# indrajeetadityaroy9/vit-inductive-bias-distillation

Hardware: AMD Instinct MI355X
Metric: distillation images/sec (BASD loss fwd+bwd+grad all-reduce), DeiT-S<-ResNet-50 @ bs256/GPU (higher is better)
Workload: dtype f32; 1 GPU; cfg2 DeiT-S<-ResNet-50 224x224; per_gpu_batch=256, global_batch=256, input_dtype=float32, layout=strided (CLS-sliced / channel-major views), backward=True, grad_allreduce_bytes=88202672, grad_allreduce=none at world size 1 (bucket packed, nothing to exchange), rank_readback=auto, readback_deferred_steps=1756, selector=basd_selector_chain mode 0, parallelism=dp1

## Files before the change

include/basd_hip.h:

```cpp
#ifndef BASD_HIP_H
#define BASD_HIP_H

#include <stdint.h>

#ifdef __cplusplus
extern "C" {
#endif

#ifndef __HIP_PLATFORM_AMD__
typedef struct ihipStream_t* hipStream_t;
#endif

#define BASD_OK 0
#define BASD_EINVAL (-1)
#define BASD_EUNSUPPORTED (-2)
#define BASD_DTYPE_F32 0
#define BASD_DTYPE_BF16 1
#define BASD_DTYPE_U8 2


int basd_gemm_nt(const void* a, int a_dtype, long a_sb, long a_sn, long a_sd, int a_rows_per_batch,
                 long a_batch_stride, const float* b, long ldb, long b_batch_stride, int M, int N, int K, int batch,
                 float* c, long ldc, long c_batch_stride, float scale, const float* bias, float beta,
                 float* colsum_part, float* col_mean, hipStream_t stream);
// ... 196 lines not shown
    const void* const* attn_ptrs;
    long a_dtype, a_sb, a_sh, a_sq, a_sk;
    const float* mix;
    long E, L, G, B, n_s, n_t, d_s, d_t, H, A, has_cls, n_a, n, max_sweeps;
    const int* atap0; const int* atap1; const float* alam;
    const int* tap0; const int* tap1; const float* lam; const int* range0; const int* range1;
    const int* g0; const int* g1; const float* glam;
    float* omega; float* omega_t; float* raw; float* mu_t; float* tc; float* mu_s; float* tr_part; float* tr_s;
    float* a_prime;
    double* g_all; double* l_all;
    float* W; float* sigma; int* jflags; int* sweeps;
    float* tr_t; float* nuc; float* loss_b; float* k_prime;
    float* h; float* dx; const float* grad_layers;
    double* g_slabs; long g_splits;
    const float* uw_ce; float* uw_out;
    void* jac_ws;
    float* w_stack; float* sigma_u;
} BasdProcrustesArgs;
int basd_procrustes_forward_fused(const BasdProcrustesArgs* args, hipStream_t stream);
int basd_procrustes_tuning(int transposed_cores);

int basd_stack_product_t(const double* la, const double* lb, long l_batch_stride, int n, int batch, int lb_period,
                         float* w, long w_batch_stride, hipStream_t stream);
int basd_kprime_from_transposed(const float* w, long w_batch_stride, const float* sigma, int n, int batch,
                                const double* lb, long l_batch_stride, int lb_period, float* z, long z_batch_stride,
                                float* k_prime, hipStream_t stream);
int basd_procrustes_finish_transposed(const float* w, long w_batch_stride, const float* sigma, int n, int n_s,
                                      int batch, int t_period ,
                                      const double* gb, long g_batch_stride, const float* omega, const int* tap0,
                                      const int* tap1, const float* lam, const float* tr_s_part, int tr_slabs,
                                      float* tr_s, float* tr_t, float* nuc, float* loss, const double* lb,
                                      long l_batch_stride, int lb_period, float* k_prime, hipStream_t stream);
int basd_procrustes_finish_tuning(int fused);
int basd_ustack_stash(const float* wc, long wc_batch_stride, int n, int batch, float* w_stack, long w_stack_stride,
                      hipStream_t stream);
int basd_ustack_from_transposed(const float* x, long x_batch_stride, const float* sigma, int n, int batch,
                                float* w_stack, long w_stack_stride, float* scratch, long scratch_batch_stride,
                                float* sigma_u, int max_sweeps, int* jflags, hipStream_t stream);

int basd_scale_unless_one(float* x, long count, const float* num, const float* den, hipStream_t stream);

int basd_cross_entropy(const void* logits, int dtype, long ld, int B, int C, const long* labels, const float* probs,
                       long pld, float label_smoothing, long ignore_index, float* row_loss, float* dlogits,
                       hipStream_t stream);


int basd_event_create(void** out);
int basd_event_destroy(void* event);
int basd_stream_wait_event(hipStream_t stream, void* event);
int basd_event_record(void* event, hipStream_t stream);
int basd_event_synchronize(void* event);
int basd_stream_create_priority(void** out, int level);
int basd_event_create_timed(void** out);
int basd_event_elapsed_ms(void* from, void* to, float* ms_out);


int basd_teacher_factor(const float* w, long w_batch_stride, const float* sigma, int n, int n_s, int batch,
                        const double* la, const double* gb, long g_batch_stride, const float* omega,
                        const int* tap0, const int* tap1, const float* lam, const int* range0, const int* range1,
                        float* kt, float* tnorm2, hipStream_t stream);
int basd_teacher_factor_tiled(const float* w, long w_batch_stride, const float* sigma, int n, int n_s, int batch,
                              const double* la, const double* gb, long g_batch_stride, const float* omega,
                              const int* tap0, const int* tap1, const float* lam, const int* range0, const int* range1,
                              float* kt, float* tnorm2, float* z_scratch, hipStream_t stream);

int basd_mix_grad_tokens(const float* r, const void* const* tok_ptrs, int dtype, int L, long sb, long sn, long sd,
// ... 89 lines not shown
```

vit-inductive-bias-distillation_amd/basd_amd/_lib.py:

```python
from __future__ import annotations

import ctypes as C
import os
import threading

_HERE = os.path.dirname(os.path.abspath(__file__))
LIB_PATH = os.path.join(_HERE, "libbasd_hip.so")

vp, i32, i64, f32, f64 = C.c_void_p, C.c_int, C.c_long, C.c_float, C.c_double

SIGNATURES = {
    "basd_gemm_nt": [vp, i32, i64, i64, i64, i32, i64, vp, i64, i64, i32, i32, i32, i32, vp, i64, i64, f32, vp, f32,
                     vp, vp, vp],
    "basd_gemm_tn_splits": [i32],
    "basd_gemm_tn": [vp, vp, i32, i64, i64, i64, i64, i64, i64, i64, i64, i32, i32, i32, i32, i32, vp, vp, i32, vp,
                     vp, i64, i64, f32, vp],
    "basd_colmean_parts": [i32],
    "basd_colmean": [vp, i32, i64, i64, i64, i32, i64, i32, i32, i32, i32, vp, vp, vp],
    "basd_colmean_multi": [vp, i32, i64, i64, i64, i32, i32, i32, i32, i32, vp, vp, i32, vp],
    "basd_syrk_splits": [i32, i32, i32],
    "basd_syrk_multi": [vp, i32, i64, i64, i64, i32, i32, i32, i32, vp, vp, i32, vp, vp, i64, i32, vp, i32, i32, vp],
    "basd_jacobi_workspace_ints": [i32, i32],
    "basd_jacobi_twopass_workspace_bytes": [i32, i32, i32],
    "basd_jacobi_stacked_twopass": [vp, i64, i32, i32, vp, i32, i32, f32, vp, vp, vp],
# ... 23 lines not shown
    "basd_grassmann_distance": [vp, i32, vp, vp, i32, vp, i32, vp, vp, vp],
    "basd_grassmann_distance_padded": [vp, i32, i32, vp, vp, i32, vp, i32, vp, vp],
    "basd_selector_tail": [vp] * 10 + [i32, i32, i32, i32] + [vp] * 14 + [vp],
    "basd_sqrt_clamp": [vp, vp, i64, vp],
    "basd_gram_finish": [vp, vp, i32, i32, i64, vp, vp, vp],
    "basd_cross_entropy": [vp, i32, i64, i32, i32, vp, vp, i64, f32, i64, vp, vp, vp],
    "basd_token_weights": [vp, i32, vp, i32, i64, i64, i64, i64, i32, i32, i32, i32, i32, i32, i32, vp, vp, vp, vp,
                           vp, vp, vp, vp, vp, vp],
    "basd_student_project": [vp, i32, i64, i64, i32, i32, i32, i32, vp, vp, vp, vp, vp, vp, vp, vp, vp, vp],
    "basd_teacher_center": [vp, i32, vp, i32, i64, i64, i64, i32, i32, i32, vp, vp, vp, vp, vp, vp, vp],
    "basd_teacher_center_multi": [vp, i32, vp, i32, i32, i64, i64, i64, i32, i32, i32, vp, vp, vp, vp, vp, vp, vp],
    "basd_teacher_center_stream_scratch_floats": [i32, i32, i32, i32],
    "basd_teacher_center_stream": [vp, i32, vp, i32, i32, i64, i64, i64, i32, i32, i32, vp, vp, vp, vp, vp, vp, vp, vp],
    "basd_gram_f64": [vp, i64, i32, i32, i32, vp, i64, vp],
    "basd_gram_f64_split": [vp, i64, i32, i32, i32, i32, vp, vp, vp],
    "basd_chol_f64": [vp, i64, i32, i32, vp, i64, vp],
    "basd_stack_product": [vp, vp, i64, i32, i32, i32, vp, i64, vp],
    "basd_procrustes_finalize": [vp, i64, vp, i32, i32, i32, i32, vp, i64, vp, vp, vp, vp, vp, i32, vp, vp, vp, vp,
                                 vp, vp],
    "basd_student_project_multi": [vp, i32, i64, i64, i32, i32, i32, i32, i32, i32, vp, i64, vp, vp, vp, vp, vp, vp,
                                   vp, vp, vp],
    "basd_student_grad_multi": [vp, i32, i64, i64, i32, i32, i32, i32, i32, vp, i64, vp, vp, vp, vp, vp, vp, f32, vp,
                                vp, vp, vp],
    "basd_student_grad_fused": [vp, i32, i64, i64, i32, i32, i32, i32, i32, i32, vp, i64, vp, vp, vp, vp, vp, vp, vp,
                                f32, vp, vp],
    "basd_procrustes_forward_fused": [vp, vp],
    "basd_procrustes_tuning": [i32],
    "basd_jacobi_plain4_fits": [i32],
    "basd_stack_product_t": [vp, vp, i64, i32, i32, i32, vp, i64, vp],
    "basd_kprime_from_transposed": [vp, i64, vp, i32, i32, vp, i64, i32, vp, i64, vp, vp],
    "basd_procrustes_finish_transposed": [vp, i64, vp, i32, i32, i32, i32, vp, i64, vp, vp, vp, vp, vp, i32, vp, vp, vp,
                                          vp, vp, i64, i32, vp, vp],
    "basd_procrustes_finish_tuning": [i32],
    "basd_ustack_stash": [vp, i64, i32, i32, vp, i64, vp],
    "basd_ustack_from_transposed": [vp, i64, vp, i32, i32, vp, i64, vp, i64, vp, i32, vp, vp],
    "basd_resample_tokens": [vp, i32, i64, i64, i64, i32, i32, i32, i32, vp, vp, vp, vp, vp],
    "basd_resample_tokens_adjoint": [vp, i32, i32, i32, i32, vp, vp, vp, vp, vp, vp, vp],
    "basd_teacher_factor": [vp, i64, vp, i32, i32, i32, vp, vp, i64, vp, vp, vp, vp, vp, vp, vp, vp, vp],
    "basd_teacher_factor_tiled": [vp, i64, vp, i32, i32, i32, vp, vp, i64, vp, vp, vp, vp, vp, vp, vp, vp, vp, vp],
    "basd_mix_grad_tokens": [vp, vp, i32, i32, i64, i64, i64, i32, i32, i32, i32, vp, vp, vp, vp, vp],
    "basd_mix_grad_tokens_scratch_floats": [i32, i32, i32, i32],
    "basd_mix_grad_tokens_onepass": [vp, vp, i32, i32, i64, i64, i64, i32, i32, i32, i32, vp, vp, vp, vp, vp, vp],
    "basd_token_weight_bwd": [vp, vp, i32, i32, i32, i32, vp, vp, vp, vp, vp, vp, i32, i32, i64, i64, i64, i64, i32,
                              i32, i32, vp, vp, vp],
    "basd_build_angle_stack": [vp, i32, vp, i32, vp, vp],
    "basd_grassmann_distance_bwd": [vp, vp, i32, vp, vp, i32, vp, vp, i32, vp, vp],
    "basd_eigvec_k2": [vp, vp, i32, i32, i32, vp, vp],
    "basd_selector_chain": [vp],
    "basd_rank_certificate": [vp, vp, i32, i32, f64, vp, vp, vp],
    "basd_rank_certificate_scratch_bytes": [i32],
    "basd_debug_fill_lds": [C.c_uint, vp],
    "basd_selector_chain_tail": [vp, i32, i32],
    "basd_jacobi_lds_square_fits": [i32],
    "basd_event_record": [vp, vp],
    "basd_event_synchronize": [vp],
    "basd_stream_create_priority": [vp, i32],
    "basd_event_create_timed": [vp],
    "basd_event_elapsed_ms": [vp, vp, vp],
    "basd_sfadamw_chunk": [],
    "basd_sfadamw_step": [vp, vp, i32, vp, i32, f32, i32, vp],
    "basd_sfadamw_swap": [vp, vp, i32, vp, i32, vp],
    "basd_sfadamw_launches": [],
    "basd_eval_batch": [vp, i32, i64, i32, i32, vp, i32, vp, f32, i32, vp, vp],
    "basd_mix_batch": [vp, i32, vp, i32, i32, i32, i32, i32, i32, f64, i32, i32, i32, i32, vp, vp, vp, i32, f64, vp,
                       vp],
    "basd_attn_importance": [vp, i32, i64, i64, i32, i32, i32, i32, i32, f32, vp, vp],
# ... 94 lines not shown
```

vit-inductive-bias-distillation_amd/csrc/fused.hip:

```cpp
#include "basd_common.h"
#include "../../include/basd_hip.h"

namespace basd {

__global__ void __launch_bounds__(256) uwso_combine_kernel(const float* __restrict__ ce, const float* __restrict__ loss_b,
                                                           int E, int B, float* __restrict__ out) {
    constexpr int CH = 32;
    __shared__ double red[CH][4];
    const int tid = threadIdx.x;
    double geo_sum = 0.;
    for (int e0 = 0; e0 < E; e0 += CH) {
        const int ne = E - e0 < CH ? E - e0 : CH;
        for (int e = 0; e < ne; ++e) {
            double acc = 0.;
            for (int b = tid; b < B; b += 256) acc += (double)loss_b[(long)(e0 + e) * B + b];
            for (int m = 32; m > 0; m >>= 1) acc += __shfl_xor(acc, m, 64);
            if ((tid & 63) == 0) red[e][tid >> 6] = acc;
        }
        __syncthreads();
        if (tid == 0)
            for (int e = 0; e < ne; ++e) {
                const float layer = (float)(((red[e][0] + red[e][1]) + (red[e][2] + red[e][3])) / (double)B);
                out[4 + E + e0 + e] = layer;
                geo_sum += (double)layer;
            }
        __syncthreads();
    }
    if (tid == 0) {
        const float c = ce[0], geo = (float)(geo_sum / (double)E);
        const float eps = 1.1920929e-7f;
        const float i0 = 1.f / fmaxf(c, eps), i1 = 1.f / fmaxf(geo, eps);
        const float w0 = i0 / (i0 + i1), w1 = i1 / (i0 + i1);
        out[0] = w0;
        out[1] = w1;
        out[2] = w0 * c + w1 * geo;
        out[3] = geo;
        for (int e = 0; e < E; ++e) out[4 + e] = w1 / (float)E;
    }
}

__global__ void __launch_bounds__(256) scale_unless_one_kernel(float* __restrict__ x, long count4, long count,
                                                               const float* __restrict__ num,
                                                               const float* __restrict__ den) {
    const float f = den ? num[0] / den[0] : num[0];
    if (f == 1.f) return;
    const long i = (long)blockIdx.x * 256 + threadIdx.x;
    if (i < count4) {
        float4 v = ((float4*)x)[i];
        v.x *= f; v.y *= f; v.z *= f; v.w *= f;
        ((float4*)x)[i] = v;
    }
    if (blockIdx.x == 0 && threadIdx.x < (int)(count - 4 * count4)) x[4 * count4 + threadIdx.x] *= f;
}

}

extern "C" {

int basd_scale_unless_one(float* x, long count, const float* num, const float* den, hipStream_t stream) {
    BASD_CHECK_ARG(x && num && count > 0 && ((uintptr_t)x & 15) == 0);
    const long count4 = count / 4;
    basd::scale_unless_one_kernel<<<(unsigned)((count4 + 255) / 256 + (count4 == 0)), 256, 0, stream>>>(x, count4, count, num, den);
    BASD_RETURN_LAST();
}

static int procrustes_tail(const BasdProcrustesArgs* a, const float* grad_layers, int E, int B, int n_s, int n, int d_s,
                           int EB, long nn, long om_stride, hipStream_t st) {
    int rc;
#define BASD_TRY(call)            \
    do {                          \
        rc = (call);              \
        if (rc != BASD_OK) return rc; \
    } while (0)
    if (a->uw_ce) {
        BASD_CHECK_ARG(a->uw_out != nullptr);
        basd::uwso_combine_kernel<<<1, 256, 0, st>>>(a->uw_ce, a->loss_b, E, B, a->uw_out);
        grad_layers = a->uw_out + 4;
    }
    if (a->dx) {
        BASD_CHECK_ARG(a->k_prime && a->h && grad_layers);
        rc = basd_student_grad_fused(a->student_ptrs, (int)a->s_dtype, a->s_sb, a->s_sn, E, B, n_s, n, d_s,
                                     (int)a->s_aligned, a->omega, om_stride, a->mu_s, a->k_prime, a->a_prime, a->tap0,
                                     a->tap1, a->lam, grad_layers, 2.0f / (float)B, a->dx, st);
        if (rc != BASD_EUNSUPPORTED) return rc;
        BASD_TRY(basd_gemm_tn(a->k_prime, a->a_prime, BASD_DTYPE_F32, 0, n, 1, nn, 0, d_s, 1, (long)n * d_s, 1 << 30, n,
                              n, d_s, EB, nullptr, nullptr, 1, nullptr, a->h, d_s, (long)n * d_s, 1.f, st));
        BASD_TRY(basd_student_grad_multi(a->student_ptrs, (int)a->s_dtype, a->s_sb, a->s_sn, E, B, n_s, n, d_s, a->omega,
                                         om_stride, a->mu_s, a->h, a->tap0, a->tap1, a->lam, grad_layers,
                                         2.0f / (float)B, a->dx, nullptr, nullptr, st));
    }
#undef BASD_TRY
    return BASD_OK;
}

static int g_transposed_cores = 1;
// ... 132 lines not shown
```

vit-inductive-bias-distillation_amd/csrc/procrustes.hip:

```cpp
#include "basd_common.h"
#include "../../include/basd_hip.h"

namespace basd {

typedef double f64x4 __attribute__((ext_vector_type(4)));

template <typename T>
__global__ void __launch_bounds__(256) token_weights_kernel(const void* const* __restrict__ attn_ptrs,
                                                            const float* __restrict__ mix, int L, long sb, long sh,
                                                            long sq, long sk, int H, int A, int has_cls, int n_a,
                                                            int n_t, int n_s, const int* __restrict__ atap0,
                                                            const int* __restrict__ atap1,
                                                            const float* __restrict__ alam,
                                                            const int* __restrict__ tap0,
                                                            const int* __restrict__ tap1,
                                                            const float* __restrict__ lam, float* __restrict__ omega,
                                                            float* __restrict__ omega_t, float* __restrict__ raw_out) {
    extern __shared__ float sm[];
    float* raw = sm;
    float* w = sm + n_a;
    __shared__ float red[32];
    const int b = blockIdx.x, tid = threadIdx.x;
    for (int j = tid; j < n_a; j += blockDim.x) {
        float acc = 0.f;
        if (has_cls) {
            for (int h = 0; h < H; ++h) {
                float m = 0.f;
                for (int l = 0; l < L; ++l)
                    m += mix[l] * ldg_f32((const BASD_GLOBAL_AS T*)attn_ptrs[l] + (b * sb + h * sh + (long)(1 + j) * sk));
                acc += m;
            }
            acc /= (float)H;
// ... 7 lines not shown
                }
            acc /= (float)(H * A);
        }
        raw[j] = acc;
        if (raw_out) raw_out[(long)b * n_a + j] = acc;
    }
    __syncthreads();
    float part = 0.f;
    for (int n = tid; n < n_s; n += blockDim.x) {
        float v;
        if (atap0) {
            const float l1 = alam[n];
            v = (1.f - l1) * raw[atap0[n]] + l1 * raw[atap1[n]];
        } else {
            v = raw[n];
        }
        w[n] = v;
        part += v;
    }
    const float total = block_sum(part, red);
    for (int n = tid; n < n_s; n += blockDim.x) {
        const float v = w[n] / total;
        w[n] = v;
        omega[(long)b * n_s + n] = v;
    }
    __syncthreads();
    for (int j = tid; j < n_t; j += blockDim.x) {
        float acc = 0.f;
        if (tap0) {
            for (int n = 0; n < n_s; ++n) {
                const float l1 = lam[n];
                if (tap0[n] == j) acc += (1.f - l1) * w[n];
                if (tap1[n] == j) acc += l1 * w[n];
            }
        } else {
            acc = w[j];
        }
        omega_t[(long)b * n_t + j] = acc;
    }
}

template <typename T>
__global__ void __launch_bounds__(256) student_project_kernel(const T* __restrict__ X, long sb, long sn, int n_s,
                                                              int n_t, int D, const float* __restrict__ omega,
                                                              const int* __restrict__ tap0,
                                                              const int* __restrict__ tap1,
                                                              const float* __restrict__ lam,
                                                              const int* __restrict__ range0,
                                                              const int* __restrict__ range1,
                                                              float* __restrict__ mu_out, float* __restrict__ tr_part,
                                                              float* __restrict__ Ap) {
    extern __shared__ float sm[];
    float* w = sm;
    __shared__ float red[4][64];
    __shared__ float mu[64];
    __shared__ float scratch[32];
    const int b = blockIdx.y, d0 = blockIdx.x * 64, tid = threadIdx.x;
    const int cl = tid & 63, rg = tid >> 6, d = d0 + cl;
    const bool live = d < D;
    const T* Xb = X + (long)b * sb + d;
    for (int n = tid; n < n_s; n += 256) w[n] = omega[(long)b * n_s + n];
    __syncthreads();
    float acc = 0.f;
    if (live)
        for (int n = rg; n < n_s; n += 4) acc = fmaf(w[n], to_f32(Xb[(long)n * sn]), acc);
    red[rg][cl] = acc;
// ... 165 lines not shown
    }
    *(float4*)(&red[rg][c4]) = acc;
    __syncthreads();
    if (tid < SP_W) {
        float m = 0.f;
#pragma unroll
        for (int q = 0; q < 32; ++q) m += red[q][tid];
        mu[tid] = m;
        if (d0 + tid < D) mu_out[((long)e * B + b) * D + d0 + tid] = m;
    }
    __syncthreads();
    const float4 m4 = *(const float4*)(mu + c4);
    float part = 0.f;
    if (live)
        for (int n = rg; n < n_s; n += 32) {
            const float4 v = *(const float4*)(xs + n * SP_W + c4);
            const float cx = v.x - m4.x, cy = v.y - m4.y, cz = v.z - m4.z, cw = v.w - m4.w;
            part = fmaf(w[n], fmaf(cx, cx, fmaf(cy, cy, fmaf(cz, cz, cw * cw))), part);
        }
    const float tr = block_sum(part, scratch);
    if (tid == 0) tr_part[((long)e * B + b) * gridDim.x + blockIdx.x] = tr;
    if (!live) return;
    float* Ab = Ap + ((long)e * B + b) * n_t * D + d0 + c4;
    for (int j = rg; j < n_t; j += 32) {
        const int n0 = range0 ? range0[j] : j, n1 = range1 ? range1[j] : j + 1;
        float4 a = make_float4(0.f, 0.f, 0.f, 0.f);
        for (int n = n0; n < n1; ++n) {
            const float cw = tap0 ? (t0[n] == j ? c0[n] : 0.f) + (t1[n] == j ? c1[n] : 0.f) : w[n];
            const float4 v = *(const float4*)(xs + n * SP_W + c4);
            a.x = fmaf(cw, v.x - m4.x, a.x); a.y = fmaf(cw, v.y - m4.y, a.y);
            a.z = fmaf(cw, v.z - m4.z, a.z); a.w = fmaf(cw, v.w - m4.w, a.w);
        }
        *(float4*)(Ab + (long)j * D) = a;
    }
}

template <typename T>
__global__ void __launch_bounds__(256) teacher_center_kernel(const void* const* __restrict__ tok_ptrs,
                                                             const float* __restrict__ mix, int L, long sb, long sn,
                                                             long sd, int n, int D, const int* __restrict__ g0,
                                                             const int* __restrict__ g1,
                                                             const float* __restrict__ glam,
                                                             const float* __restrict__ omega_t,
                                                             float* __restrict__ mu_out, float* __restrict__ Tc) {
    extern __shared__ float sm[];
    float* tile = sm;
    float* wt = sm + (size_t)n * 65;
    float* mu = wt + n;
    const int b = blockIdx.y, d0 = blockIdx.x * 64, tid = threadIdx.x;
    for (int j = tid; j < n; j += 256) wt[j] = omega_t[(long)b * n + j];
    const int total = n * 64;
    const bool feat_fast = sd == 1;
    for (int idx = tid; idx < total; idx += 256) {
        int j, dd;
        if (feat_fast) { j = idx >> 6; dd = idx & 63; }
        else { dd = idx / n; j = idx - dd * n; }
        const int d = d0 + dd;
        float v = 0.f;
        if (d < D) {
            const long off = b * sb + (long)d * sd;
            if (g0) {
                const long r0 = g0[j], r1 = g1[j];
                float a0 = 0.f, a1 = 0.f;
                for (int l = 0; l < L; ++l) {
                    const BASD_GLOBAL_AS T* p = (const BASD_GLOBAL_AS T*)tok_ptrs[l];
                    a0 = fmaf(mix[l], ldg_f32(p + (off + r0 * sn)), a0);
                    a1 = fmaf(mix[l], ldg_f32(p + (off + r1 * sn)), a1);
                }
                const float l1 = glam[j];
                v = (1.f - l1) * a0 + l1 * a1;
            } else {
                for (int l = 0; l < L; ++l)
                    v = fmaf(mix[l], ldg_f32((const BASD_GLOBAL_AS T*)tok_ptrs[l] + (off + (long)j * sn)), v);
            }
        }
        tile[j * 65 + dd] = v;
    }
    __syncthreads();
    if (tid < 64) {
        float acc = 0.f;
        for (int j = 0; j < n; ++j) acc = fmaf(wt[j], tile[j * 65 + tid], acc);
        mu[tid] = acc;
        if (d0 + tid < D) mu_out[(long)b * D + d0 + tid] = acc;
    }
    __syncthreads();
    float* out = Tc + (long)b * n * D;
    for (int idx = tid; idx < total; idx += 256) {
        const int j = idx >> 6, dd = idx & 63, d = d0 + dd;
        if (d < D) out[(long)j * D + d] = tile[j * 65 + dd] - mu[dd];
    }
}

constexpr int TCM_W = 16, TCM_G = 4;
template <typename T>
__global__ void __launch_bounds__(256) teacher_center_multi_kernel(
    const void* const* __restrict__ tok_ptrs, const float* __restrict__ mix, int L, int G, long sb, long sn, long sd,
    int n, int D, const int* __restrict__ g0, const int* __restrict__ g1, const float* __restrict__ glam,
    const float* __restrict__ omega_t, float* __restrict__ mu_out, float* __restrict__ Tc) {
    extern __shared__ float sm[];
    const int B = gridDim.y, b = blockIdx.y, d0 = blockIdx.x * TCM_W, tid = threadIdx.x;
    float* tile = sm;
    float* wt = sm + (size_t)G * n * (TCM_W + 1);
    float* mu = wt + (size_t)G * n;
    for (int idx = tid; idx < G * n; idx += 256) {
        const int g = idx / n, j = idx - g * n;
        wt[idx] = omega_t[((long)g * B + b) * n + j];
    }
    const int total = n * TCM_W;
    const bool feat_fast = sd == 1;
    for (int idx = tid; idx < total; idx += 256) {
        int j, dd;
        if (feat_fast) { j = idx / TCM_W; dd = idx - j * TCM_W; }
        else { dd = idx / n; j = idx - dd * n; }
        const int d = d0 + dd;
        float v[TCM_G] = {0.f, 0.f, 0.f, 0.f};
        if (d < D) {
            const long off = b * sb + (long)d * sd;
            if (g0) {
                const long r0 = g0[j], r1 = g1[j];
                const float l1 = glam[j], l0 = 1.f - l1;
                for (int l = 0; l < L; ++l) {
                    const BASD_GLOBAL_AS T* p = (const BASD_GLOBAL_AS T*)tok_ptrs[l];
                    const float x = l0 * ldg_f32(p + (off + r0 * sn)) + l1 * ldg_f32(p + (off + r1 * sn));
#pragma unroll
                    for (int g = 0; g < TCM_G; ++g)
// ... 922 lines not shown
    const T* x0 = X + (long)b * sb + (long)i0 * sn;
    const T* x1 = X + (long)b * sb + (long)i1 * sn;
    float* o = out + ((long)b * n_out + s) * D;
    for (int d = threadIdx.x; d < D; d += 128) o[d] = l0 * to_f32(x0[(long)d * sd]) + l1 * to_f32(x1[(long)d * sd]);
}

__global__ void __launch_bounds__(128) resample_tokens_adjoint_kernel(const float* __restrict__ dY, int n_in,
                                                                      int n_out, int D,
                                                                      const int* __restrict__ tap0,
                                                                      const int* __restrict__ tap1,
                                                                      const float* __restrict__ lam,
                                                                      const int* __restrict__ range0,
                                                                      const int* __restrict__ range1,
                                                                      float* __restrict__ dX) {
    const int j = blockIdx.x, b = blockIdx.y;
    const int s0 = range0[j], s1 = range1[j];
    for (int d = threadIdx.x; d < D; d += 128) {
        float acc = 0.f;
        for (int s = s0; s < s1; ++s) {
            const float l1 = lam[s];
            const float coef = (tap0[s] == j ? 1.f - l1 : 0.f) + (tap1[s] == j ? l1 : 0.f);
            acc = fmaf(coef, dY[((long)b * n_out + s) * D + d], acc);
        }
        dX[((long)b * n_in + j) * D + d] = acc;
    }
}

}

using namespace basd;

extern "C" {

int basd_token_weights(const void* const* attn_ptrs, int dtype, const float* mix, int L, long sb, long sh, long sq,
                       long sk, int B, int H, int A, int has_cls, int n_a, int n_t, int n_s, const int* atap0,
                       const int* atap1, const float* alam, const int* tap0, const int* tap1, const float* lam,
                       float* omega, float* omega_t, float* raw_out, hipStream_t stream) {
    BASD_CHECK_ARG(attn_ptrs && mix && omega && omega_t && L > 0 && B > 0 && H > 0 && n_a > 0 && n_t > 0 && n_s > 0);
    BASD_CHECK_ARG(A == n_a + (has_cls ? 1 : 0));
    BASD_CHECK_ARG((n_a == n_s) == (atap0 == nullptr));
    BASD_CHECK_ARG((n_t == n_s) == (tap0 == nullptr));
    const size_t lds = sizeof(float) * (size_t)(n_a + n_s);
    if (dtype == BASD_DTYPE_F32)
        token_weights_kernel<float><<<B, 256, lds, stream>>>(attn_ptrs, mix, L, sb, sh, sq, sk, H, A, has_cls, n_a, n_t, n_s, atap0, atap1, alam, tap0, tap1, lam, omega, omega_t, raw_out);
    else if (dtype == BASD_DTYPE_BF16)
        token_weights_kernel<__hip_bfloat16><<<B, 256, lds, stream>>>(attn_ptrs, mix, L, sb, sh, sq, sk, H, A, has_cls, n_a, n_t, n_s, atap0, atap1, alam, tap0, tap1, lam, omega, omega_t, raw_out);
    else
        return BASD_EINVAL;
    BASD_RETURN_LAST();
}

int basd_student_project(const void* x, int dtype, long sb, long sn, int B, int n_s, int n_t, int D,
                         const float* omega, const int* tap0, const int* tap1, const float* lam, const int* range0,
                         const int* range1, float* mu, float* tr_s, float* a_prime, hipStream_t stream) {
    BASD_CHECK_ARG(x && omega && mu && tr_s && a_prime && B > 0 && n_s > 0 && n_t > 0 && D > 0);
    BASD_CHECK_ARG((n_t == n_s) == (tap0 == nullptr));
    const size_t lds = sizeof(float) * (size_t)n_s;
    const dim3 grid((D + 63) / 64, B);
    const int esz = dtype == BASD_DTYPE_F32 ? 4 : 2;
    const size_t lds_slab = sizeof(float) * (size_t)n_s * 65;
    const bool staged = D % 4 == 0 && ((uintptr_t)x * 1) % 16 == 0 && (sb * esz) % 16 == 0 && (sn * esz) % 16 == 0 &&
                        (esz == 4 || D % 8 == 0) && lds_slab <= 64 * 1024;
    if (dtype == BASD_DTYPE_F32) {
        if (staged) {
            (void)hipFuncSetAttribute((const void*)student_project_lds_kernel<float>, hipFuncAttributeMaxDynamicSharedMemorySize, (int)lds_slab);
            student_project_lds_kernel<float><<<grid, 256, lds_slab, stream>>>((const float*)x, sb, sn, n_s, n_t, D, omega, tap0, tap1, lam, range0, range1, mu, tr_s, a_prime);
        } else {
            student_project_kernel<float><<<grid, 256, lds, stream>>>((const float*)x, sb, sn, n_s, n_t, D, omega, tap0, tap1, lam, range0, range1, mu, tr_s, a_prime);
        }
    } else if (dtype == BASD_DTYPE_BF16) {
        if (staged) {
            (void)hipFuncSetAttribute((const void*)student_project_lds_kernel<__hip_bfloat16>, hipFuncAttributeMaxDynamicSharedMemorySize, (int)lds_slab);
            student_project_lds_kernel<__hip_bfloat16><<<grid, 256, lds_slab, stream>>>((const __hip_bfloat16*)x, sb, sn, n_s, n_t, D, omega, tap0, tap1, lam, range0, range1, mu, tr_s, a_prime);
        } else {
            student_project_kernel<__hip_bfloat16><<<grid, 256, lds, stream>>>((const __hip_bfloat16*)x, sb, sn, n_s, n_t, D, omega, tap0, tap1, lam, range0, range1, mu, tr_s, a_prime);
        }
    } else {
        return BASD_EINVAL;
    }
    BASD_RETURN_LAST();
}

int basd_teacher_center(const void* const* tok_ptrs, int dtype, const float* mix, int L, long sb, long sn, long sd,
                        int B, int n, int D, const int* g0, const int* g1, const float* glam, const float* omega_t,
                        float* mu, float* tc, hipStream_t stream) {
    BASD_CHECK_ARG(tok_ptrs && mix && omega_t && mu && tc && L > 0 && B > 0 && n > 0 && D > 0);
    BASD_CHECK_ARG((g0 == nullptr) == (g1 == nullptr) && (g0 == nullptr) == (glam == nullptr));
    const size_t lds = sizeof(float) * ((size_t)n * 65 + n + 64);
    if (lds > 150 * 1024) return BASD_EUNSUPPORTED;
    const dim3 grid((D + 63) / 64, B);
    if (dtype == BASD_DTYPE_F32) {
        (void)hipFuncSetAttribute((const void*)teacher_center_kernel<float>, hipFuncAttributeMaxDynamicSharedMemorySize, 150 * 1024);
        teacher_center_kernel<float><<<grid, 256, lds, stream>>>(tok_ptrs, mix, L, sb, sn, sd, n, D, g0, g1, glam, omega_t, mu, tc);
    } else if (dtype == BASD_DTYPE_BF16) {
        (void)hipFuncSetAttribute((const void*)teacher_center_kernel<__hip_bfloat16>, hipFuncAttributeMaxDynamicSharedMemorySize, 150 * 1024);
        teacher_center_kernel<__hip_bfloat16><<<grid, 256, lds, stream>>>(tok_ptrs, mix, L, sb, sn, sd, n, D, g0, g1, glam, omega_t, mu, tc);
    } else {
        return BASD_EINVAL;
    }
    BASD_RETURN_LAST();
}

int basd_teacher_center_multi(const void* const* tok_ptrs, int dtype, const float* mix, int L, int G, long sb, long sn,
                              long sd, int B, int n, int D, const int* g0, const int* g1, const float* glam,
                              const float* omega_t, float* mu, float* tc, hipStream_t stream) {
    BASD_CHECK_ARG(tok_ptrs && mix && omega_t && mu && tc && L > 0 && G > 0 && B > 0 && n > 0 && D > 0);
    BASD_CHECK_ARG((g0 == nullptr) == (g1 == nullptr) && (g0 == nullptr) == (glam == nullptr));
    BASD_CHECK_ARG(B <= 65535);
    const size_t lds = sizeof(float) * ((size_t)G * n * (TCM_W + 1) + (size_t)G * n + (size_t)G * TCM_W);
    if (G > TCM_G || lds > 150 * 1024) return BASD_EUNSUPPORTED;
    const dim3 grid((D + TCM_W - 1) / TCM_W, B);
    if (dtype == BASD_DTYPE_F32) {
        (void)hipFuncSetAttribute((const void*)teacher_center_multi_kernel<float>, hipFuncAttributeMaxDynamicSharedMemorySize, 150 * 1024);
        teacher_center_multi_kernel<float><<<grid, 256, lds, stream>>>(tok_ptrs, mix, L, G, sb, sn, sd, n, D, g0, g1, glam, omega_t, mu, tc);
    } else if (dtype == BASD_DTYPE_BF16) {
        (void)hipFuncSetAttribute((const void*)teacher_center_multi_kernel<__hip_bfloat16>, hipFuncAttributeMaxDynamicSharedMemorySize, 150 * 1024);
        teacher_center_multi_kernel<__hip_bfloat16><<<grid, 256, lds, stream>>>(tok_ptrs, mix, L, G, sb, sn, sd, n, D, g0, g1, glam, omega_t, mu, tc);
    } else {
        return BASD_EINVAL;
    }
    BASD_RETURN_LAST();
}

// ... 266 lines not shown
    const size_t lds = sizeof(float) * (size_t)n_t * (SG_W + SG_LD);
    const dim3 grid((D + SG_W - 1) / SG_W, B, E);
#define LAUNCH_SGF(TY, RP)                                                                                           \
    student_grad_fused_kernel<TY, RP><<<grid, 256, lds, stream>>>(x_ptrs, sb, sn, n_s, n_t, D, omega, omega_e_stride, mu, \
                                                                  k_prime, a_prime, tap0, tap1, lam, scale_ptr,      \
                                                                  scale_const, dx)
#define LAUNCH_SGF_T(TY)                 \
    do {                                 \
        if (rp <= 4) LAUNCH_SGF(TY, 4);  \
        else if (rp <= 8) LAUNCH_SGF(TY, 8);  \
        else if (rp <= 13) LAUNCH_SGF(TY, 13); \
        else LAUNCH_SGF(TY, 16);         \
    } while (0)
    if (dtype == BASD_DTYPE_F32) LAUNCH_SGF_T(float);
    else if (dtype == BASD_DTYPE_BF16) LAUNCH_SGF_T(__hip_bfloat16);
    else return BASD_EINVAL;
#undef LAUNCH_SGF_T
#undef LAUNCH_SGF
    BASD_RETURN_LAST();
}

int basd_student_project_multi(const void* const* x_ptrs, int dtype, long sb, long sn, int E, int B, int n_s, int n_t,
                               int D, int ptrs_16B_aligned, const float* omega, long omega_e_stride, const int* tap0,
                               const int* tap1, const float* lam, const int* range0, const int* range1, float* mu,
                               float* tr_s, float* a_prime, hipStream_t stream) {
    BASD_CHECK_ARG(x_ptrs && omega && mu && tr_s && a_prime && E > 0 && B > 0 && n_s > 0 && n_t > 0 && D > 0);
    BASD_CHECK_ARG((n_t == n_s) == (tap0 == nullptr));
    BASD_CHECK_ARG(E <= 65535 && B <= 65535);
    const int esz = dtype == BASD_DTYPE_F32 ? 4 : 2;
    const size_t lds = sizeof(float) * ((size_t)n_s * SP_W + 5 * (size_t)n_s);
    const bool ok = ptrs_16B_aligned && D % 4 == 0 && (sb * esz) % 16 == 0 && (sn * esz) % 16 == 0 &&
                    (esz == 4 || D % 8 == 0) && lds <= 96 * 1024;
    if (!ok) return BASD_EUNSUPPORTED;
    const dim3 grid((D + SP_W - 1) / SP_W, B, E);
    if (dtype == BASD_DTYPE_F32) {
        (void)hipFuncSetAttribute((const void*)student_project_v4_kernel<float>, hipFuncAttributeMaxDynamicSharedMemorySize, (int)lds);
        student_project_v4_kernel<float><<<grid, 256, lds, stream>>>(x_ptrs, sb, sn, n_s, n_t, D, omega, omega_e_stride, tap0, tap1, lam, range0, range1, mu, tr_s, a_prime);
    } else if (dtype == BASD_DTYPE_BF16) {
        (void)hipFuncSetAttribute((const void*)student_project_v4_kernel<__hip_bfloat16>, hipFuncAttributeMaxDynamicSharedMemorySize, (int)lds);
        student_project_v4_kernel<__hip_bfloat16><<<grid, 256, lds, stream>>>(x_ptrs, sb, sn, n_s, n_t, D, omega, omega_e_stride, tap0, tap1, lam, range0, range1, mu, tr_s, a_prime);
    } else {
        return BASD_EINVAL;
    }
    BASD_RETURN_LAST();
}

int basd_resample_tokens(const void* x, int dtype, long sb, long sn, long sd, int B, int n_in, int n_out, int D,
                         const int* tap0, const int* tap1, const float* lam, float* out, hipStream_t stream) {
    BASD_CHECK_ARG(x && tap0 && tap1 && lam && out && B > 0 && n_in > 0 && n_out > 0 && D > 0);
    const dim3 grid(n_out, B);
    if (dtype == BASD_DTYPE_F32)
        resample_tokens_kernel<float><<<grid, 128, 0, stream>>>((const float*)x, sb, sn, sd, n_in, n_out, D, tap0, tap1, lam, out);
    else if (dtype == BASD_DTYPE_BF16)
        resample_tokens_kernel<__hip_bfloat16><<<grid, 128, 0, stream>>>((const __hip_bfloat16*)x, sb, sn, sd, n_in, n_out, D, tap0, tap1, lam, out);
    else
        return BASD_EINVAL;
    BASD_RETURN_LAST();
}

int basd_resample_tokens_adjoint(const float* dy, int B, int n_in, int n_out, int D, const int* tap0,
                                 const int* tap1, const float* lam, const int* range0, const int* range1, float* dx,
                                 hipStream_t stream) {
    BASD_CHECK_ARG(dy && tap0 && tap1 && lam && range0 && range1 && dx && B > 0 && n_in > 0 && n_out > 0 && D > 0);
    resample_tokens_adjoint_kernel<<<dim3(n_in, B), 128, 0, stream>>>(dy, n_in, n_out, D, tap0, tap1, lam, range0, range1, dx);
    BASD_RETURN_LAST();
}

// ... 2 lines not shown
```

Before: 170,300 images/s.

## Add persistent prefetching student projection and vectorized teacher centering kernels

Replaces the per-slab student projection launch with a persistent grid-stride kernel. It prefetches the next work item's tokens into registers while the current item computes, and sizes the grid from occupancy. Teacher centering gets a vectorized variant that uses float4 loads for aligned feature-major and channel-major layouts, plus float4 stores. Also added are an LDS-staged token-weight kernel (opt-in, off by default) and a capped grid-stride scale kernel. The goal is to hide global-memory latency and cut launch and tail cost in the loss front end. In exchange it adds more code paths and register pressure from the prefetch buffers, and its performance depends on the occupancy query.

```diff
diff --git a/include/basd_hip.h b/include/basd_hip.h
--- a/include/basd_hip.h
+++ b/include/basd_hip.h
@@ -252,6 +252,8 @@
                                       float* tr_s, float* tr_t, float* nuc, float* loss, const double* lb,
                                       long l_batch_stride, int lb_period, float* k_prime, hipStream_t stream);
 int basd_procrustes_finish_tuning(int fused);
+int basd_procrustes_front_tuning(int staged);
+int basd_procrustes_front_grid(int max_blocks);
 int basd_ustack_stash(const float* wc, long wc_batch_stride, int n, int batch, float* w_stack, long w_stack_stride,
                       hipStream_t stream);
 int basd_ustack_from_transposed(const float* x, long x_batch_stride, const float* sigma, int n, int batch,
diff --git a/vit-inductive-bias-distillation_amd/basd_amd/_lib.py b/vit-inductive-bias-distillation_amd/basd_amd/_lib.py
--- a/vit-inductive-bias-distillation_amd/basd_amd/_lib.py
+++ b/vit-inductive-bias-distillation_amd/basd_amd/_lib.py
@@ -79,6 +79,8 @@
     "basd_procrustes_finish_transposed": [vp, i64, vp, i32, i32, i32, i32, vp, i64, vp, vp, vp, vp, vp, i32, vp, vp, vp,
                                           vp, vp, i64, i32, vp, vp],
     "basd_procrustes_finish_tuning": [i32],
+    "basd_procrustes_front_tuning": [i32],
+    "basd_procrustes_front_grid": [i32],
     "basd_ustack_stash": [vp, i64, i32, i32, vp, i64, vp],
     "basd_ustack_from_transposed": [vp, i64, vp, i32, i32, vp, i64, vp, i64, vp, i32, vp, vp],
     "basd_resample_tokens": [vp, i32, i64, i64, i64, i32, i32, i32, i32, vp, vp, vp, vp, vp],
diff --git a/vit-inductive-bias-distillation_amd/csrc/fused.hip b/vit-inductive-bias-distillation_amd/csrc/fused.hip
--- a/vit-inductive-bias-distillation_amd/csrc/fused.hip
+++ b/vit-inductive-bias-distillation_amd/csrc/fused.hip
@@ -44,8 +44,7 @@
                                                                const float* __restrict__ den) {
     const float f = den ? num[0] / den[0] : num[0];
     if (f == 1.f) return;
-    const long i = (long)blockIdx.x * 256 + threadIdx.x;
-    if (i < count4) {
+    for (long i = (long)blockIdx.x * 256 + threadIdx.x; i < count4; i += (long)gridDim.x * 256) {
         float4 v = ((float4*)x)[i];
         v.x *= f; v.y *= f; v.z *= f; v.w *= f;
         ((float4*)x)[i] = v;
@@ -60,7 +59,8 @@
 int basd_scale_unless_one(float* x, long count, const float* num, const float* den, hipStream_t stream) {
     BASD_CHECK_ARG(x && num && count > 0 && ((uintptr_t)x & 15) == 0);
     const long count4 = count / 4;
-    basd::scale_unless_one_kernel<<<(unsigned)((count4 + 255) / 256 + (count4 == 0)), 256, 0, stream>>>(x, count4, count, num, den);
+    const long blocks = (count4 + 255) / 256 + (count4 == 0);
+    basd::scale_unless_one_kernel<<<(unsigned)(blocks < 2048 ? blocks : 2048), 256, 0, stream>>>(x, count4, count, num, den);
     BASD_RETURN_LAST();
 }
 
diff --git a/vit-inductive-bias-distillation_amd/csrc/procrustes.hip b/vit-inductive-bias-distillation_amd/csrc/procrustes.hip
--- a/vit-inductive-bias-distillation_amd/csrc/procrustes.hip
+++ b/vit-inductive-bias-distillation_amd/csrc/procrustes.hip
@@ -1,3 +1,4 @@
+#include <atomic>
 #include "basd_common.h"
 #include "../../include/basd_hip.h"
 
@@ -71,6 +72,102 @@
                 const float l1 = lam[n];
                 if (tap0[n] == j) acc += (1.f - l1) * w[n];
                 if (tap1[n] == j) acc += l1 * w[n];
+            }
+        } else {
+            acc = w[j];
+        }
+        omega_t[(long)b * n_t + j] = acc;
+    }
+}
+
+template <typename T>
+__global__ void __launch_bounds__(256) token_weights_staged_kernel(
+    const void* const* __restrict__ attn_ptrs, const float* __restrict__ mix, int L, long sb, long sh, long sq, long sk,
+    int H, int A, int has_cls, int n_a, int n_t, int n_s, const int* __restrict__ atap0, const int* __restrict__ atap1,
+    const float* __restrict__ alam, const int* __restrict__ tap0, const int* __restrict__ tap1,
+    const float* __restrict__ lam, float* __restrict__ omega, float* __restrict__ omega_t, float* __restrict__ raw_out,
+    int chunk_rows) {
+    extern __shared__ float sm[];
+    float* raw = sm;
+    float* w = raw + n_a;
+    float* s_alam = w + n_s;
+    int* s_at0 = (int*)(s_alam + (atap0 ? n_s : 0));
+    int* s_at1 = s_at0 + (atap0 ? n_s : 0);
+    float* s_lam = (float*)(s_at1 + (atap0 ? n_s : 0));
+    int* s_t0 = (int*)(s_lam + (tap0 ? n_s : 0));
+    int* s_t1 = s_t0 + (tap0 ? n_s : 0);
+    float* s_mix = (float*)(s_t1 + (tap0 ? n_s : 0));
+    float* stage = s_mix + L;
+    __shared__ float red[32];
+    const int b = blockIdx.x, tid = threadIdx.x, lane = tid & 63, wid = tid >> 6;
+    for (int n = tid; n < n_s; n += 256) {
+        if (atap0) { s_alam[n] = alam[n]; s_at0[n] = atap0[n]; s_at1[n] = atap1[n]; }
+        if (tap0) { s_lam[n] = lam[n]; s_t0[n] = tap0[n]; s_t1[n] = tap1[n]; }
+    }
+    for (int l = tid; l < L; l += 256) s_mix[l] = mix[l];
+    for (int j = tid; j < n_a; j += 256) raw[j] = 0.f;
+    const int nrows = has_cls ? H : H * A;
+    for (int r0 = 0; r0 < nrows; r0 += chunk_rows) {
+        const int nr = nrows - r0 < chunk_rows ? nrows - r0 : chunk_rows;
+        __syncthreads();
+        for (int p = wid; p < nr * L; p += 4) {
+            const int rr = p / L, l = p - rr * L, r = r0 + rr;
+            long off = b * sb;
+            if (has_cls) {
+                off += r * sh + sk;
+            } else {
+                const int h = r / A;
+                off += h * sh + (r - h * A) * sq;
+            }
+            const BASD_GLOBAL_AS T* src = (const BASD_GLOBAL_AS T*)attn_ptrs[l] + off;
+            float* dst = stage + (long)p * n_a;
+            for (int j = lane; j < n_a; j += 64) dst[j] = ldg_f32(src + (long)j * sk);
+        }
+        __syncthreads();
+        for (int j = tid; j < n_a; j += 256) {
+            float acc = raw[j];
+            for (int rr = 0; rr < nr; ++rr) {
+                float m = 0.f;
+                for (int l = 0; l < L; ++l) m += s_mix[l] * stage[((long)rr * L + l) * n_a + j];
+                acc += m;
+            }
+            raw[j] = acc;
+        }
+    }
+    for (int j = tid; j < n_a; j += 256) {
+        float acc = raw[j];
+        if (has_cls) acc /= (float)H;
+        else acc /= (float)(H * A);
+        raw[j] = acc;
+        if (raw_out) raw_out[(long)b * n_a + j] = acc;
+    }
+    __syncthreads();
+    float part = 0.f;
+    for (int n = tid; n < n_s; n += blockDim.x) {
+        float v;
+        if (atap0) {
+            const float l1 = s_alam[n];
+            v = (1.f - l1) * raw[s_at0[n]] + l1 * raw[s_at1[n]];
+        } else {
+            v = raw[n];
+        }
+        w[n] = v;
+        part += v;
+    }
+    const float total = block_sum(part, red);
+    for (int n = tid; n < n_s; n += blockDim.x) {
+        const float v = w[n] / total;
+        w[n] = v;
+        omega[(long)b * n_s + n] = v;
+    }
+    __syncthreads();
+    for (int j = tid; j < n_t; j += blockDim.x) {
+        float acc = 0.f;
+        if (tap0) {
+            for (int n = 0; n < n_s; ++n) {
+                const float l1 = s_lam[n];
+                if (s_t0[n] == j) acc += (1.f - l1) * w[n];
+                if (s_t1[n] == j) acc += l1 * w[n];
             }
         } else {
             acc = w[j];
@@ -302,6 +399,123 @@
             a.z = fmaf(cw, v.z - m4.z, a.z); a.w = fmaf(cw, v.w - m4.w, a.w);
         }
         *(float4*)(Ab + (long)j * D) = a;
+    }
+}
+
+constexpr int SP_PF = 8;
+template <typename T>
+__global__ void __launch_bounds__(256) student_project_pipe_kernel(const void* const* __restrict__ x_ptrs, long sb,
+                                                                   long sn, int n_s, int n_t, int D,
+                                                                   const float* __restrict__ omega,
+                                                                   long omega_e_stride, const int* __restrict__ tap0,
+                                                                   const int* __restrict__ tap1,
+                                                                   const float* __restrict__ lam,
+                                                                   const int* __restrict__ range0,
+                                                                   const int* __restrict__ range1,
+                                                                   float* __restrict__ mu_out,
+                                                                   float* __restrict__ tr_part,
+                                                                   float* __restrict__ Ap, int nslab, int B,
+                                                                   int items) {
+    extern __shared__ __attribute__((aligned(16))) float sm[];
+    float* xs = sm;
+    float* w = sm + (long)n_s * SP_W;
+    float* c0 = w + n_s;
+    float* c1 = c0 + n_s;
+    int* t0 = (int*)(c1 + n_s);
+    int* t1 = t0 + n_s;
+    int* r0s = t1 + n_s;
+    int* r1s = r0s + n_t;
+    __shared__ __attribute__((aligned(16))) float red[32][SP_W];
+    __shared__ __attribute__((aligned(16))) float mu[SP_W];
+    __shared__ float scratch[32];
+    const int tid = threadIdx.x, fq = tid & 7, rg = tid >> 3, c4 = 4 * fq;
+    const bool has_row = tid < n_s;
+    float l1 = 0.f;
+    if (tap0 && has_row) {
+        l1 = lam[tid];
+        t0[tid] = tap0[tid];
+        t1[tid] = tap1[tid];
+    }
+    if (range0)
+        for (int j = tid; j < n_t; j += 256) {
+            r0s[j] = range0[j];
+            r1s[j] = range1[j];
+        }
+    float4 pf[SP_PF];
+    float wpf = 0.f;
+    auto fetch = [&](int it) {
+        const int slab = it % nslab, be = it / nslab, b = be % B, e = be / B;
+        const bool lv = slab * SP_W + c4 < D;
+        const BASD_GLOBAL_AS T* Xb = (const BASD_GLOBAL_AS T*)x_ptrs[e] + (long)b * sb + slab * SP_W;
+#pragma unroll
+        for (int q = 0; q < SP_PF; ++q) {
+            const int n = rg + 32 * q;
+            pf[q] = make_float4(0.f, 0.f, 0.f, 0.f);
+            if (lv && n < n_s) pf[q] = ld4f(Xb + (long)n * sn + c4);
+        }
+        if (has_row) wpf = omega[(long)e * omega_e_stride + (long)b * n_s + tid];
+    };
+    int item = blockIdx.x;
+    if (item < items) fetch(item);
+    for (; item < items; item += gridDim.x) {
+        const int slab = item % nslab, be = item / nslab, b = be % B, e = be / B, d0 = slab * SP_W;
+        const bool live = d0 + c4 < D;
+#pragma unroll
+        for (int q = 0; q < SP_PF; ++q) {
+            const int n = rg + 32 * q;
+            if (n < n_s) *(float4*)(xs + n * SP_W + c4) = pf[q];
+        }
+        if (has_row) {
+            w[tid] = wpf;
+            if (tap0) {
+                c0[tid] = (1.f - l1) * wpf;
+                c1[tid] = l1 * wpf;
+            }
+        }
+        __syncthreads();
+        if (item + (int)gridDim.x < items) fetch(item + (int)gridDim.x);
+        float4 acc = make_float4(0.f, 0.f, 0.f, 0.f);
+        for (int n = rg; n < n_s; n += 32) {
+            const float4 v = *(const float4*)(xs + n * SP_W + c4);
+            const float wn = w[n];
+            acc.x = fmaf(wn, v.x, acc.x); acc.y = fmaf(wn, v.y, acc.y);
+            acc.z = fmaf(wn, v.z, acc.z); acc.w = fmaf(wn, v.w, acc.w);
+        }
+        *(float4*)(&red[rg][c4]) = acc;
+        __syncthreads();
+        if (tid < SP_W) {
+            float m = 0.f;
+#pragma unroll
+            for (int q = 0; q < 32; ++q) m += red[q][tid];
+            mu[tid] = m;
+            if (d0 + tid < D) mu_out[((long)e * B + b) * D + d0 + tid] = m;
+        }
+        __syncthreads();
+        const float4 m4 = *(const float4*)(mu + c4);
+        float part = 0.f;
+        if (live)
+            for (int n = rg; n < n_s; n += 32) {
+                const float4 v = *(const float4*)(xs + n * SP_W + c4);
+                const float cx = v.x - m4.x, cy = v.y - m4.y, cz = v.z - m4.z, cw = v.w - m4.w;
+                part = fmaf(w[n], fmaf(cx, cx, fmaf(cy, cy, fmaf(cz, cz, cw * cw))), part);
+            }
+        const float tr = block_sum(part, scratch);
+        if (tid == 0) tr_part[((long)e * B + b) * nslab + slab] = tr;
+        if (live) {
+            float* Ab = Ap + ((long)e * B + b) * n_t * D + d0 + c4;
+            for (int j = rg; j < n_t; j += 32) {
+                const int n0 = range0 ? r0s[j] : j, n1 = range1 ? r1s[j] : j + 1;
+                float4 a = make_float4(0.f, 0.f, 0.f, 0.f);
+                for (int n = n0; n < n1; ++n) {
+                    const float cw = tap0 ? (t0[n] == j ? c0[n] : 0.f) + (t1[n] == j ? c1[n] : 0.f) : w[n];
+                    const float4 v = *(const float4*)(xs + n * SP_W + c4);
+                    a.x = fmaf(cw, v.x - m4.x, a.x); a.y = fmaf(cw, v.y - m4.y, a.y);
+                    a.z = fmaf(cw, v.z - m4.z, a.z); a.w = fmaf(cw, v.w - m4.w, a.w);
+                }
+                *(float4*)(Ab + (long)j * D) = a;
+            }
+        }
+        __syncthreads();
     }
 }
 
@@ -361,6 +575,133 @@
     }
 }
 
+template <typename T>
+__global__ void __launch_bounds__(256) teacher_center_vec_kernel(const void* const* __restrict__ tok_ptrs,
+                                                                 const float* __restrict__ mix, int L, long sb, long sn,
+                                                                 long sd, int n, int D, const int* __restrict__ g0,
+                                                                 const int* __restrict__ g1,
+                                                                 const float* __restrict__ glam,
+                                                                 const float* __restrict__ omega_t,
+                                                                 float* __restrict__ mu_out, float* __restrict__ Tc,
+                                                                 int layout, int vec_store) {
+    extern __shared__ float sm[];
+    float* tile = sm;
+    float* wt = sm + (size_t)n * 65;
+    float* mu = wt + n;
+    const int b = blockIdx.y, d0 = blockIdx.x * 64, tid = threadIdx.x;
+    for (int j = tid; j < n; j += 256) wt[j] = omega_t[(long)b * n + j];
+    const int total = n * 64;
+    const int nd = D - d0 < 64 ? D - d0 : 64;
+    if (layout)
+        for (int l = 0; l < L; ++l)
+            if ((uintptr_t)tok_ptrs[l] & 15) layout = 0;
+    if (layout == 1) {
+        for (int idx = tid; idx < n * 16; idx += 256) {
+            const int j = idx >> 4, c4 = (idx & 15) * 4;
+            float4 v = make_float4(0.f, 0.f, 0.f, 0.f);
+            if (c4 < nd) {
+                const long off = b * sb + (long)j * sn + d0 + c4;
+                for (int l = 0; l < L; ++l) {
+                    const float4 x = ld4f((const BASD_GLOBAL_AS T*)tok_ptrs[l] + off);
+                    const float ml = mix[l];
+                    v.x = fmaf(ml, x.x, v.x); v.y = fmaf(ml, x.y, v.y);
+                    v.z = fmaf(ml, x.z, v.z); v.w = fmaf(ml, x.w, v.w);
+                }
+            }
+            float* t = tile + j * 65 + c4;
+            t[0] = v.x; t[1] = v.y; t[2] = v.z; t[3] = v.w;
+        }
+    } else if (layout == 2) {
+        const int run = nd * n;
+        const long base = b * sb + (long)d0 * n;
+        const int qs = 1024 / n, rs = 1024 - qs * n;
+        int f = 4 * tid, dd = f / n, j = f - dd * n;
+        for (; f < total; f += 1024) {
+            float v[4] = {0.f, 0.f, 0.f, 0.f};
+            if (f + 3 < run) {
+                float4 a = make_float4(0.f, 0.f, 0.f, 0.f);
+                for (int l = 0; l < L; ++l) {
+                    const float4 x = ld4f((const BASD_GLOBAL_AS T*)tok_ptrs[l] + (base + f));
+                    const float ml = mix[l];
+                    a.x = fmaf(ml, x.x, a.x); a.y = fmaf(ml, x.y, a.y);
+                    a.z = fmaf(ml, x.z, a.z); a.w = fmaf(ml, x.w, a.w);
+                }
+                v[0] = a.x; v[1] = a.y; v[2] = a.z; v[3] = a.w;
+            } else {
+#pragma unroll
+                for (int c = 0; c < 4; ++c)
+                    if (f + c < run)
+                        for (int l = 0; l < L; ++l)
+                            v[c] = fmaf(mix[l], ldg_f32((const BASD_GLOBAL_AS T*)tok_ptrs[l] + (base + f + c)), v[c]);
+            }
+            int jj = j, d = dd;
+#pragma unroll
+            for (int c = 0; c < 4; ++c) {
+                tile[jj * 65 + d] = v[c];
+                if (++jj == n) { jj = 0; ++d; }
+            }
+            j += rs; dd += qs;
+            if (j >= n) { j -= n; ++dd; }
+        }
+    } else {
+        const bool feat_fast = sd == 1;
+        const int qs = 256 / n, rs = 256 - qs * n;
+        int dd = feat_fast ? tid & 63 : tid / n, j = feat_fast ? tid >> 6 : tid - dd * n;
+        for (int idx = tid; idx < total; idx += 256) {
+            const int d = d0 + dd;
+            float v = 0.f;
+            if (d < D) {
+                const long off = b * sb + (long)d * sd;
+                if (g0) {
+                    const long r0 = g0[j], r1 = g1[j];
+                    float a0 = 0.f, a1 = 0.f;
+                    for (int l = 0; l < L; ++l) {
+                        const BASD_GLOBAL_AS T* p = (const BASD_GLOBAL_AS T*)tok_ptrs[l];
+                        a0 = fmaf(mix[l], ldg_f32(p + (off + r0 * sn)), a0);
+                        a1 = fmaf(mix[l], ldg_f32(p + (off + r1 * sn)), a1);
+                    }
+                    const float l1 = glam[j];
+                    v = (1.f - l1) * a0 + l1 * a1;
+                } else {
+                    for (int l = 0; l < L; ++l)
+                        v = fmaf(mix[l], ldg_f32((const BASD_GLOBAL_AS T*)tok_ptrs[l] + (off + (long)j * sn)), v);
+                }
+            }
+            tile[j * 65 + dd] = v;
+            if (feat_fast) {
+                j += 4;
+            } else {
+                j += rs; dd += qs;
+                if (j >= n) { j -= n; ++dd; }
+            }
+        }
+    }
+    __syncthreads();
+    if (tid < 64) {
+        float acc = 0.f;
+        for (int j = 0; j < n; ++j) acc = fmaf(wt[j], tile[j * 65 + tid], acc);
+        mu[tid] = acc;
+        if (d0 + tid < D) mu_out[(long)b * D + d0 + tid] = acc;
+    }
+    __syncthreads();
+    float* out = Tc + (long)b * n * D;
+    if (vec_store) {
+        for (int idx = tid; idx < n * 16; idx += 256) {
+            const int j = idx >> 4, c4 = (idx & 15) * 4;
+            if (c4 < nd) {
+                const float* t = tile + j * 65 + c4;
+                *(float4*)(out + (long)j * D + d0 + c4) =
+                    make_float4(t[0] - mu[c4], t[1] - mu[c4 + 1], t[2] - mu[c4 + 2], t[3] - mu[c4 + 3]);
+            }
+        }
+    } else {
+        for (int idx = tid; idx < total; idx += 256) {
+            const int j = idx >> 6, dd = idx & 63, d = d0 + dd;
+            if (d < D) out[(long)j * D + d] = tile[j * 65 + dd] - mu[dd];
+        }
+    }
+}
+
 constexpr int TCM_W = 16, TCM_G = 4;
 template <typename T>
 __global__ void __launch_bounds__(256) teacher_center_multi_kernel(
@@ -1349,6 +1690,36 @@
 
 extern "C" {
 
+static int g_front_new = 2;
+static int g_front_grid = 0;
+int basd_procrustes_front_tuning(int staged) {
+    const int prev = g_front_new;
+    if (staged >= 0) g_front_new = staged > 2 ? 2 : staged;
+    return prev;
+}
+int basd_procrustes_front_grid(int max_blocks) {
+    const int prev = g_front_grid;
+    if (max_blocks >= 0) g_front_grid = max_blocks;
+    return prev;
+}
+
+static int student_pipe_resident(int dtype, size_t lds) {
+    static std::atomic<long> cached_lds[2]{{-1}, {-1}};
+    static std::atomic<int> cached_grid[2]{{0}, {0}};
+    const int k = dtype == BASD_DTYPE_F32 ? 0 : 1;
+    if (cached_lds[k].load(std::memory_order_acquire) == (long)lds) return cached_grid[k].load(std::memory_order_relaxed);
+    int dev = 0, cus = 0, per_cu = 0, grid = 1024;
+    const void* fn = k == 0 ? (const void*)student_project_pipe_kernel<float>
+                            : (const void*)student_project_pipe_kernel<__hip_bfloat16>;
+    if (hipGetDevice(&dev) == hipSuccess &&
+        hipDeviceGetAttribute(&cus, hipDeviceAttributeMultiprocessorCount, dev) == hipSuccess &&
+        hipOccupancyMaxActiveBlocksPerMultiprocessor(&per_cu, fn, 256, lds) == hipSuccess && cus > 0 && per_cu > 0)
+        grid = per_cu * cus;
+    cached_grid[k].store(grid, std::memory_order_relaxed);
+    cached_lds[k].store((long)lds, std::memory_order_release);
+    return grid;
+}
+
 int basd_token_weights(const void* const* attn_ptrs, int dtype, const float* mix, int L, long sb, long sh, long sq,
                        long sk, int B, int H, int A, int has_cls, int n_a, int n_t, int n_s, const int* atap0,
                        const int* atap1, const float* alam, const int* tap0, const int* tap1, const float* lam,
@@ -1358,6 +1729,20 @@
     BASD_CHECK_ARG((n_a == n_s) == (atap0 == nullptr));
     BASD_CHECK_ARG((n_t == n_s) == (tap0 == nullptr));
     const size_t lds = sizeof(float) * (size_t)(n_a + n_s);
+    if (dtype != BASD_DTYPE_F32 && dtype != BASD_DTYPE_BF16) return BASD_EINVAL;
+    const size_t fixed = (size_t)n_a + n_s + (atap0 ? 3 * (size_t)n_s : 0) + (tap0 ? 3 * (size_t)n_s : 0) + L;
+    const size_t budget = 48 * 1024 / sizeof(float), per_row = (size_t)L * n_a;
+    if (g_front_new == 1 && fixed + per_row <= budget) {
+        const size_t nrows = has_cls ? (size_t)H : (size_t)H * A;
+        size_t rows = (budget - fixed) / per_row;
+        if (rows > nrows) rows = nrows;
+        const size_t lds_st = sizeof(float) * (fixed + rows * per_row);
+        if (dtype == BASD_DTYPE_F32)
+            token_weights_staged_kernel<float><<<B, 256, lds_st, stream>>>(attn_ptrs, mix, L, sb, sh, sq, sk, H, A, has_cls, n_a, n_t, n_s, atap0, atap1, alam, tap0, tap1, lam, omega, omega_t, raw_out, (int)rows);
+        else
+            token_weights_staged_kernel<__hip_bfloat16><<<B, 256, lds_st, stream>>>(attn_ptrs, mix, L, sb, sh, sq, sk, H, A, has_cls, n_a, n_t, n_s, atap0, atap1, alam, tap0, tap1, lam, omega, omega_t, raw_out, (int)rows);
+        BASD_RETURN_LAST();
+    }
     if (dtype == BASD_DTYPE_F32)
         token_weights_kernel<float><<<B, 256, lds, stream>>>(attn_ptrs, mix, L, sb, sh, sq, sk, H, A, has_cls, n_a, n_t, n_s, atap0, atap1, alam, tap0, tap1, lam, omega, omega_t, raw_out);
     else if (dtype == BASD_DTYPE_BF16)
@@ -1406,6 +1791,23 @@
     const size_t lds = sizeof(float) * ((size_t)n * 65 + n + 64);
     if (lds > 150 * 1024) return BASD_EUNSUPPORTED;
     const dim3 grid((D + 63) / 64, B);
+    if (g_front_new && (dtype == BASD_DTYPE_F32 || dtype == BASD_DTYPE_BF16)) {
+        const long esz = dtype == BASD_DTYPE_F32 ? 4 : 2;
+        int layout = 0;
+        if (!g0 && (sb * esz) % 16 == 0) {
+            if (sd == 1 && D % 4 == 0 && (sn * esz) % 16 == 0) layout = 1;
+            else if (sn == 1 && sd == n) layout = 2;
+        }
+        const int vec_store = D % 4 == 0 && ((uintptr_t)tc & 15) == 0;
+        if (dtype == BASD_DTYPE_F32) {
+            (void)hipFuncSetAttribute((const void*)teacher_center_vec_kernel<float>, hipFuncAttributeMaxDynamicSharedMemorySize, 150 * 1024);
+            teacher_center_vec_kernel<float><<<grid, 256, lds, stream>>>(tok_ptrs, mix, L, sb, sn, sd, n, D, g0, g1, glam, omega_t, mu, tc, layout, vec_store);
+        } else {
+            (void)hipFuncSetAttribute((const void*)teacher_center_vec_kernel<__hip_bfloat16>, hipFuncAttributeMaxDynamicSharedMemorySize, 150 * 1024);
+            teacher_center_vec_kernel<__hip_bfloat16><<<grid, 256, lds, stream>>>(tok_ptrs, mix, L, sb, sn, sd, n, D, g0, g1, glam, omega_t, mu, tc, layout, vec_store);
+        }
+        BASD_RETURN_LAST();
+    }
     if (dtype == BASD_DTYPE_F32) {
         (void)hipFuncSetAttribute((const void*)teacher_center_kernel<float>, hipFuncAttributeMaxDynamicSharedMemorySize, 150 * 1024);
         teacher_center_kernel<float><<<grid, 256, lds, stream>>>(tok_ptrs, mix, L, sb, sn, sd, n, D, g0, g1, glam, omega_t, mu, tc);
@@ -1738,7 +2140,26 @@
     const bool ok = ptrs_16B_aligned && D % 4 == 0 && (sb * esz) % 16 == 0 && (sn * esz) % 16 == 0 &&
                     (esz == 4 || D % 8 == 0) && lds <= 96 * 1024;
     if (!ok) return BASD_EUNSUPPORTED;
-    const dim3 grid((D + SP_W - 1) / SP_W, B, E);
+    if (dtype != BASD_DTYPE_F32 && dtype != BASD_DTYPE_BF16) return BASD_EINVAL;
+    const int nslab = (D + SP_W - 1) / SP_W;
+    if (g_front_new && n_s <= 32 * SP_PF && (long)nslab * B * E <= 0x7fffffffL) {
+        const int items = nslab * B * E;
+        const size_t lds_v4 = lds;
+        const size_t lds = lds_v4 + (range0 ? sizeof(int) * 2 * (size_t)n_t : 0);
+        if (dtype == BASD_DTYPE_F32)
+            (void)hipFuncSetAttribute((const void*)student_project_pipe_kernel<float>, hipFuncAttributeMaxDynamicSharedMemorySize, (int)lds);
+        else
+            (void)hipFuncSetAttribute((const void*)student_project_pipe_kernel<__hip_bfloat16>, hipFuncAttributeMaxDynamicSharedMemorySize, (int)lds);
+        int blocks = student_pipe_resident(dtype, lds);
+        if (g_front_grid > 0 && blocks > g_front_grid) blocks = g_front_grid;
+        if (blocks > items) blocks = items;
+        if (dtype == BASD_DTYPE_F32)
+            student_project_pipe_kernel<float><<<blocks, 256, lds, stream>>>(x_ptrs, sb, sn, n_s, n_t, D, omega, omega_e_stride, tap0, tap1, lam, range0, range1, mu, tr_s, a_prime, nslab, B, items);
+        else
+            student_project_pipe_kernel<__hip_bfloat16><<<blocks, 256, lds, stream>>>(x_ptrs, sb, sn, n_s, n_t, D, omega, omega_e_stride, tap0, tap1, lam, range0, range1, mu, tr_s, a_prime, nslab, B, items);
+        BASD_RETURN_LAST();
+    }
+    const dim3 grid(nslab, B, E);
     if (dtype == BASD_DTYPE_F32) {
         (void)hipFuncSetAttribute((const void*)student_project_v4_kernel<float>, hipFuncAttributeMaxDynamicSharedMemorySize, (int)lds);
         student_project_v4_kernel<float><<<grid, 256, lds, stream>>>(x_ptrs, sb, sn, n_s, n_t, D, omega, omega_e_stride, tap0, tap1, lam, range0, range1, mu, tr_s, a_prime);
```

Result: slower. 161,100 images/s (-5.4%).
